# AbrahamSanders/realtime-codec-agent

Measured on AMD Instinct MI355X. Metric: batch-encode audio-hours/hour (+ xRT and p50 frame-step latency of 1 duplex stream in `duplex`), higher is better.
Workload: dtype f32; 1 GPU; batch MagiCodec-style encode, 16 kHz stereo, 0.1 s chunks / 2.0 s context, 256 windows per step (BASELINE configs[1]); codebook=131072x16

## Files before the change

### realtime_codec_agent_amd/csrc/rca_codec.hip

```cpp
#include <stdarg.h>

#include <algorithm>
#include <array>
#include <cmath>
#include <map>
#include <type_traits>

#include "rca_common.h"

namespace rca {
thread_local char g_err[512] = {0};
}
using namespace rca;

typedef float f32x16 __attribute__((ext_vector_type(16)));

#define RCA_LAT_MAX_FRAMES 64
#define RCA_LDS_BUDGET (152 * 1024)

typedef float f32x4 __attribute__((ext_vector_type(4)));

struct RowSrc {
    const float* base;
    int C;
// ... 1508 lines not shown
            cinit[4 * g + 0] = h4.x; cinit[4 * g + 1] = h4.y; cinit[4 * g + 2] = h4.z; cinit[4 * g + 3] = h4.w;
        }
#pragma unroll
        for (int ft = 0; ft < FN; ++ft) {
            f32x16 acc = cinit;
#pragma unroll
            for (int kp = 0; kp < 8; ++kp) acc = __builtin_amdgcn_mfma_f32_32x32x2f32(av[kp], zb[ft][kp], acc, 0, 0, 0);
#pragma unroll
            for (int r = 0; r < 16; ++r) {
                const unsigned c = (unsigned)(c0 + (r & 3) + 8 * (r >> 2) + 4 * half);
                if (acc[r] > best[ft]) { best[ft] = acc[r]; bidx[ft] = c; }
            }
        }
    }
    __shared__ unsigned long long red[FN][4][32];
#pragma unroll
    for (int ft = 0; ft < FN; ++ft) {
        unsigned long long key = bidx[ft] == 0xFFFFFFFFu ? 0ull : pack_key(best[ft], bidx[ft]);
        const unsigned long long other = __shfl_xor(key, 32);
        key = other > key ? other : key;
        if (lane < 32) red[ft][wave][lane] = key;
    }
    __syncthreads();
    for (int i = threadIdx.x; i < FN * 32; i += 256) {
        const int ft = i >> 5, l = i & 31;
        const long f = f0 + i;
        if (f < F) {
            unsigned long long key = red[ft][0][l];
            for (int w = 1; w < 4; ++w) key = red[ft][w][l] > key ? red[ft][w][l] : key;
            atomicMax(&keys[f], key);
        }
    }
}

struct RowDst {
    int64_t* base;
    int C;
    long chan_stride;
    long win_stride;
    int fc;
    const long* row_off = nullptr;
};
__global__ __launch_bounds__(256) void vq_finalize_kernel(unsigned long long* __restrict__ keys, RowDst dst, long rows) {
    const long i = (long)blockIdx.x * blockDim.x + threadIdx.x;
    if (i >= rows) return;
    const unsigned long long key = keys[i];
    keys[i] = 0ull;
    const long b = i / dst.fc;
    const int j = (int)(i - b * dst.fc);
    dst.base[(dst.row_off ? dst.row_off[b] : (b % dst.C) * dst.chan_stride + (b / dst.C) * dst.win_stride) + j] =
        key == 0ull ? (int64_t)0 : (int64_t)(0xFFFFFFFFu - (unsigned)(key & 0xFFFFFFFFull));
}

__global__ __launch_bounds__(256) void embed_codes_kernel(const int64_t* __restrict__ codes, long ldc, const float* __restrict__ cb,
                                                          float* __restrict__ zq, int B, int F, int J, int N,
                                                          int* __restrict__ err) {
    const long idx = (long)blockIdx.x * blockDim.x + threadIdx.x;
    if (idx >= (long)B * J * F) return;
    const int f = (int)(idx % F);
    const long r = idx / F;
    const int j = (int)(r % J);
    const int b = (int)(r / J);
    int64_t c = codes[(long)b * ldc + f];
    if (c < 0 || c >= N) { atomicExch(err, 1); c = 0; }
    zq[idx] = cb[c * J + j];
}

__global__ __launch_bounds__(256) void transpose_fj_kernel(const float* __restrict__ in, float* __restrict__ out, int B,
                                                           int F, int J) {
    const long idx = (long)blockIdx.x * blockDim.x + threadIdx.x;
    if (idx >= (long)B * J * F) return;
    const int f = (int)(idx % F);
    const long r = idx / F;
    const int j = (int)(r % J);
    const int b = (int)(r / J);
    out[idx] = in[((long)b * F + f) * J + j];
}
__global__ __launch_bounds__(256) void transpose_df_kernel(const float* __restrict__ in, float* __restrict__ out, int B,
                                                           int D, int F) {
    const long idx = (long)blockIdx.x * blockDim.x + threadIdx.x;
    if (idx >= (long)B * D * F) return;
    const int d = (int)(idx % D);
    const long r = idx / D;
    const int f = (int)(r % F);
    const int b = (int)(r / F);
    out[idx] = in[((long)b * D + d) * F + f];
}

struct ConvLayer {
    int cin, cout, k, s, pre, tr;
    float* w = nullptr;
    float* b = nullptr;
    float* bp = nullptr;
    float* wp = nullptr;
    int K = 0, Kpad = 0, cout_pad = 0, nchunks = 0;
    float* wp2 = nullptr;
    int nchunks2 = 0;
    float* wp_tr = nullptr;
    float* w_lat = nullptr;
    int nchunks_tr = 0;
};

#ifdef RCA_CONV_SMALLCHUNK
#define RCA_CIC_K8 2
#define RCA_CIC_K16 1
#else
// ... 297 lines not shown
    return;
#endif
#pragma unroll
    for (int wn = 0; wn < 4; ++wn)
#pragma unroll
    for (int wm = 0; wm < WMT; ++wm) {
        const int t = n0 + wn_w * 128 + wn * 32 + n;
        if (t >= Lout) continue;
        if (OUT == 1) {
            float* yr = y_f32 + ((long)b * Cout + co0 + wm * 32 + 4 * half) * Lout + t;
#pragma unroll
            for (int r = 0; r < 16; ++r) yr[(long)((r & 3) + 8 * (r >> 2)) * Lout] = acc[wm][wn][r];
        } else {
            const int Cbo = Cout / 16;
#pragma unroll
            for (int g = 0; g < 4; ++g) {
                float v[4];
#pragma unroll
                for (int j = 0; j < 4; ++j) {
                    const float a = acc[wm][wn][4 * g + j];
                    v[j] = act ? fmaxf(a, a * slope) : a;
                }
                const int ch = co0 + wm * 32 + 8 * g + 4 * half;
                const long o = (((long)b * Cbo + ch / 16) * Lout + t) * 16 + (ch & 15);
                const unsigned h0 = conv_pack_bf16x2(v[0], v[1]), h1 = conv_pack_bf16x2(v[2], v[3]);
                *reinterpret_cast<uint2*>(y_hi + o) = make_uint2(h0, h1);
                if (SPLIT) {
                    const unsigned l0 = conv_pack_bf16x2(v[0] - __uint_as_float(h0 << 16), v[1] - __uint_as_float(h0 & 0xffff0000u));
                    const unsigned l1 = conv_pack_bf16x2(v[2] - __uint_as_float(h1 << 16), v[3] - __uint_as_float(h1 & 0xffff0000u));
                    *reinterpret_cast<uint2*>(y_lo + o) = make_uint2(l0, l1);
                }
            }
        }
    }
}

struct Bf16Pack { conv_bf16raw* hi = nullptr; conv_bf16raw* lo = nullptr; float* w_in8 = nullptr; };

struct rca_codec {
    rca_codec_config_t cfg;
    int device = 0;
    hipStream_t stream = nullptr;
    int hop = 1;
    int variant = 1;
    int mfma_mode = 0;
    bool lat_mode = false;
    int enc_left_frames = 0, dec_left_frames = 0;
    bool window_trim = false;
    std::vector<ConvLayer> enc, dec;
    std::vector<Bf16Pack> bf16_packs;
    bool bf16_blk_split = true;
    float *q_in_w = nullptr, *q_in_b = nullptr;
    float *cb = nullptr, *hc = nullptr, *cbp = nullptr;
    DevBuf act[2], zbuf, keys, io_a, io_b, tail;
    void* pin = nullptr; size_t pin_cap = 0;
    struct StreamGraph { hipGraphExec_t exec = nullptr; int seen = 0; unsigned long long sig = 0; };
    std::map<std::array<int, 5>, StreamGraph> sgraphs;
    bool stream_graphs = true;
    int* err_flag = nullptr;
    hipStream_t last_stream = nullptr;
    bool last_stream_valid = false;
    hipEvent_t xev = nullptr;
    struct Prof { hipEvent_t a, b; int kclass; double flops, bytes; };
    bool profile = false;
    std::vector<Prof> prof;
    std::vector<Prof> prof_pool;
};

struct ProfScope {
    rca_codec* h; hipStream_t st; rca_codec::Prof p; bool on;
    ProfScope(rca_codec* h_, hipStream_t st_, int kclass, double flops, double bytes) : h(h_), st(st_), on(h_->profile) {
        if (!on) return;
        if (!h->prof_pool.empty()) { p = h->prof_pool.back(); h->prof_pool.pop_back(); }
        else { (void)hipEventCreate(&p.a); (void)hipEventCreate(&p.b); }
        p.kclass = kclass; p.flops = flops; p.bytes = bytes;
        (void)hipEventRecord(p.a, st);
    }
    ~ProfScope() {
        if (!on) return;
        (void)hipEventRecord(p.b, st);
        h->prof.push_back(p);
    }
};

static int upload(const rca_tensor_t* ts, int n, const std::string& name, long numel, float** out) {
    const rca_tensor_t* t = find_tensor(ts, n, name);
    if (!t) return fail(RCA_ERR_MISSING, "tensor '%s' missing", name.c_str());
    if (t->numel != numel) return fail(RCA_ERR_ARG, "tensor '%s': numel %ld, expected %ld", name.c_str(), (long)t->numel, numel);
    if (t->dtype != RCA_F32) return fail(RCA_ERR_ARG, "tensor '%s' must be f32", name.c_str());
    RCA_HIP(hipMalloc((void**)out, (size_t)numel * sizeof(float)));
    RCA_HIP(hipMemcpy(*out, t->data, (size_t)numel * sizeof(float), hipMemcpyHostToDevice));
    return RCA_OK;
}

static int pack_weights_cic(const float* w_host, const ConvLayer& L, int cic, float** out, int* nchunks_out) {
    const int K = L.cin * L.k;
    const int nchunks = (L.cin + cic - 1) / cic;
    const int Kpad = nchunks * cic * L.k;
    const int cout_pad = (L.cout + 127) / 128 * 128;
    const long n = (long)(cout_pad / 32) * (Kpad / 8) * 64 * 4;
    std::vector<float> p((size_t)n, 0.0f);
    for (int cot = 0; cot < cout_pad / 32; ++cot)
        for (int q = 0; q < Kpad / 8; ++q)
            for (int lane = 0; lane < 64; ++lane)
                for (int e = 0; e < 4; ++e) {
                    const int co = cot * 32 + (lane & 31);
                    const int k = 2 * (4 * q + e) + (lane >> 5);
// ... 56 lines not shown

extern "C" const char* rca_last_error(void) { return g_err; }
extern "C" const char* rca_version(void) { return "rca-hip 0.1 (gfx950)"; }
extern "C" int rca_device_sync(int32_t device) {
    RCA_HIP(hipSetDevice(device));
    RCA_HIP(hipDeviceSynchronize());
    return RCA_OK;
}

extern "C" int rca_device_count(int* n) {
    if (!n) return fail(RCA_ERR_ARG, "null");
    RCA_HIP(hipGetDeviceCount(n));
    return RCA_OK;
}

extern "C" int rca_codec_destroy(rca_codec_t* h) {
#ifdef RCA_CONV_TIMELINE
    if (h && getenv("RCA_CONV_TIMELINE_OUT")) {
        long* b = nullptr;
        unsigned n = 6 << 16;
        (void)hipDeviceSynchronize();
        (void)hipMemcpyFromSymbol(&b, HIP_SYMBOL(rca_prof_buf), 8);
        if (b) {
            std::vector<long> host((size_t)(6 << 16) * 8);
            (void)hipMemcpy(host.data(), b, host.size() * 8, hipMemcpyDeviceToHost);
            if (FILE* f = fopen(getenv("RCA_CONV_TIMELINE_OUT"), "wb")) { fwrite(&n, 4, 1, f); fwrite(host.data(), 8, host.size(), f); fclose(f); }
        }
    }
#endif

    if (!h) return RCA_OK;
    (void)hipSetDevice(h->device);
    for (auto& pk : h->bf16_packs) {
        if (pk.hi) (void)hipFree(pk.hi);
        if (pk.lo) (void)hipFree(pk.lo);
        if (pk.w_in8) (void)hipFree(pk.w_in8);
    }
    for (auto* v : {&h->enc, &h->dec})
        for (auto& L : *v) {
            if (L.w) (void)hipFree(L.w);
            if (L.b) (void)hipFree(L.b);
            if (L.bp) (void)hipFree(L.bp);
            if (L.wp) (void)hipFree(L.wp);
            if (L.wp2) (void)hipFree(L.wp2);
            if (L.wp_tr) (void)hipFree(L.wp_tr);
            if (L.w_lat) (void)hipFree(L.w_lat);
        }
    for (float* p : {h->q_in_w, h->q_in_b, h->cb, h->hc, h->cbp})
        if (p) (void)hipFree(p);
    if (h->err_flag) (void)hipFree(h->err_flag);
    for (auto& kv : h->sgraphs)
        if (kv.second.exec) (void)hipGraphExecDestroy(kv.second.exec);
    if (h->pin) (void)hipHostFree(h->pin);
    h->act[0].release(); h->act[1].release(); h->zbuf.release(); h->keys.release(); h->io_a.release(); h->io_b.release(); h->tail.release();
    for (auto* v : {&h->prof, &h->prof_pool})
        for (auto& p : *v) { (void)hipEventDestroy(p.a); (void)hipEventDestroy(p.b); }
    if (h->xev) (void)hipEventDestroy(h->xev);
    if (h->stream) (void)hipStreamDestroy(h->stream);
    delete h;
    return RCA_OK;
}

static void codec_receptive_field(const rca_codec_config_t& c, int hop, int* enc_left, int* dec_left) {
    const int n = c.n_stages;
    long lo = 0;
    lo = lo - (c.k_latent - 1 + 1) / 2;
    for (int i = n - 1; i >= 0; --i) { const int s = c.strides[i], k = 2 * s; lo = lo * s - (k - s + 1) / 2; }
    lo = lo - (c.k_in - 1 + 1) / 2;
    *enc_left = (int)((-lo + hop - 1) / hop);
    auto ceil_div = [](long a, long b) { return a >= 0 ? (a + b - 1) / b : -((-a) / b); };
    long u = 0;
    u = u - (c.k_in - 1 + 1) / 2;
    for (int i = 0; i < n; ++i) { const int s = c.strides[i], k = 2 * s; u = ceil_div(u + (k - s + 1) / 2 - (k - 1), s); }
    u = u - (c.k_latent - 1 + 1) / 2;
    *dec_left = (int)(-u);
}

extern "C" int rca_codec_create(const rca_codec_config_t* cfg, const rca_tensor_t* ts, int32_t nt, int32_t device,
                                rca_codec_t** out) {
    if (!cfg || !ts || !out) return fail(RCA_ERR_ARG, "null argument");
    if (cfg->n_stages < 1 || cfg->n_stages > RCA_MAX_STAGES) return fail(RCA_ERR_ARG, "n_stages out of range");
    if (cfg->codebook_dim != 16) return fail(RCA_ERR_ARG, "codebook_dim must be 16 (got %d)", cfg->codebook_dim);
    if (cfg->codebook_size % 128 != 0) return fail(RCA_ERR_ARG, "codebook_size must be a multiple of 128");
    if (cfg->k_in != 7 && cfg->k_in != 3 && cfg->k_in != 5) return fail(RCA_ERR_ARG, "k_in must be 3, 5 or 7");
    if (!(cfg->leaky_slope > 0.0f && cfg->leaky_slope < 1.0f)) return fail(RCA_ERR_ARG, "leaky_slope must be in (0, 1)");
    RCA_HIP(hipSetDevice(device));
    rca_codec* h = new rca_codec();
    h->cfg = *cfg;
    h->device = device;
    int rc = RCA_OK;
    auto bail = [&](int code) { rca_codec_destroy(h); return code; };
    if (hipStreamCreateWithFlags(&h->stream, hipStreamNonBlocking) != hipSuccess) return bail(fail(RCA_ERR_HIP, "stream create"));
    const int n = cfg->n_stages;
    h->hop = 1;
    for (int i = 0; i < n; ++i) h->hop *= cfg->strides[i];
    codec_receptive_field(*cfg, h->hop, &h->enc_left_frames, &h->dec_left_frames);

    auto add = [&](std::vector<ConvLayer>& v, const std::string& name, int cin, int cout, int k, int s, int pre, int tr,
                   bool pack) -> int {
        ConvLayer L;
        L.cin = cin; L.cout = cout; L.k = k; L.s = s; L.pre = pre; L.tr = tr;
        if ((rc = upload(ts, nt, name + ".weight", (long)cin * cout * k, &L.w)) != RCA_OK) return rc;
        if ((rc = upload(ts, nt, name + ".bias", cout, &L.b)) != RCA_OK) { v.push_back(L); return rc; }
        {
            const size_t nb = ((size_t)cout + 127) / 128 * 128 + 64;
            if (hipMalloc((void**)&L.bp, nb * 4) != hipSuccess || hipMemset(L.bp, 0, nb * 4) != hipSuccess ||
                hipMemcpy(L.bp, L.b, (size_t)cout * 4, hipMemcpyDeviceToDevice) != hipSuccess) {
// ... 507 lines not shown
        const int Lout = L / E1.s;
        {
            ProfScope ps(h, st, 0, 2.0 * E1.cin * E1.k * E1.cout * (double)B * Lout + 2.0 * E0.k * E0.cout * (double)B * L,
                         4.0 * ((double)B * src.T + (double)B * E1.cout * Lout + (double)E1.cin * E1.k * E1.cout));
            prev_post = handoff(2, Lout);
            const int act = (E1.pre ? 1 : 0) | (prev_post ? 2 : 0);
            if (h->variant == 2 && try_conv_ws(E1, nullptr, y, B, L, Lout, slope, st, &fin)) { rc = RCA_OK; RCA_LAUNCH_CHECK(); }
            else if (E1.k == 4) rc = launch_conv_mfma<4, 2, 4>(E1, nullptr, y, B, L, Lout, slope, st, &fin, act, h->mfma_mode);
            else if (E1.k == 8) rc = launch_conv_mfma<8, 4, RCA_CIC_K8>(E1, nullptr, y, B, L, Lout, slope, st, &fin, act, h->mfma_mode);
            else rc = launch_conv_mfma<16, 8, RCA_CIC_K16>(E1, nullptr, y, B, L, Lout, slope, st, &fin, act, h->mfma_mode);
        }
        if (rc != RCA_OK) return rc;
        L = Lout;
        first = 2;
        if (tap_layer == 1) RCA_HIP(hipMemcpyAsync(tap_dev, y, (size_t)B * E1.cout * L * 4, hipMemcpyDeviceToDevice, st));
    } else if (h->lat_mode && !src.row_off && src.win_stride == 0 && src.C == B &&
               try_conv_lds(h, h->enc[0], src.base, src.chan_stride, src.T, h->act[cur].as<float>(), B, L, 0, st)) {
        RCA_LAUNCH_CHECK();
    } else {
        const ConvLayer& L0 = h->enc[0];
        const long total = (long)B * L;
        float* y = h->act[cur].as<float>();
        ProfScope ps(h, st, 2, 2.0 * L0.k * L0.cout * (double)total, 4.0 * ((double)total + (double)total * L0.cout));
        if (L0.k == 7) conv_in_kernel<7><<<cdiv(total, 256), 256, 0, st>>>(src, L0.w, L0.b, y, B, L0.cout, L);
        else if (L0.k == 5) conv_in_kernel<5><<<cdiv(total, 256), 256, 0, st>>>(src, L0.w, L0.b, y, B, L0.cout, L);
        else conv_in_kernel<3><<<cdiv(total, 256), 256, 0, st>>>(src, L0.w, L0.b, y, B, L0.cout, L);
        RCA_LAUNCH_CHECK();
        if (tap_layer == 0) RCA_HIP(hipMemcpyAsync(tap_dev, y, (size_t)B * L0.cout * L * 4, hipMemcpyDeviceToDevice, st));
    }
    for (size_t li = first; li < h->enc.size(); ++li) {
        const ConvLayer& Ly = h->enc[li];
        float* x = h->act[cur].as<float>();
        float* y = h->act[cur ^ 1].as<float>();
        bool done = false;
        int view = 0;
        if (li + 1 == h->enc.size() && Fz_out && keep > 0 && tap_layer < 0 && !Ly.tr) {
            const char* hk = getenv("RCA_HEAD_KEEP");
            const int want = keep + conv_view_halo(Ly);
            if (!(hk && hk[0] == '0') && want < L / Ly.s && conv_view_ok(h, Ly, B, L, want)) view = want;
        }
        if ((rc = run_conv(h, Ly, x, y, B, L, 0, st, prev_post, handoff(li + 1, L / Ly.s), &done, view)) != RCA_OK) return rc;
        if (view) *Fz_out = view;
        prev_post = done;
        L /= Ly.s;
        cur ^= 1;
        if (tap_layer == (int)li) RCA_HIP(hipMemcpyAsync(tap_dev, y, (size_t)B * Ly.cout * L * 4, hipMemcpyDeviceToDevice, st));
    }
    *ze_out = h->act[cur].as<float>();
    *F_out = F;
    return RCA_OK;
}

static int run_quantize(rca_codec* h, const float* ze, int ze_is_rows, int B, int F, int f0, int fc, RowDst dst, hipStream_t st,
                        float* ztap_dev) {
    const rca_codec_config_t& c = h->cfg;
    const long rows = (long)B * fc;
    const int J = c.codebook_dim, N = c.codebook_size;
    int rc;
    if ((rc = h->zbuf.ensure((size_t)rows * J * 4)) != RCA_OK) return rc;
    const size_t need_keys = (size_t)rows;
    if (h->keys.cap < need_keys * 8) {
        if ((rc = h->keys.ensure(need_keys * 8)) != RCA_OK) return rc;
        RCA_HIP(hipMemsetAsync(h->keys.p, 0, h->keys.cap, st));
    }
    float* z = h->zbuf.as<float>();
    in_proj_kernel<<<cdiv(rows * J, 256), 256, 0, st>>>(ze, h->q_in_w, h->q_in_b, z, B, c.latent_dim, F, f0, fc, J, ze_is_rows);
    RCA_LAUNCH_CHECK();
    if (ztap_dev) RCA_HIP(hipMemcpyAsync(ztap_dev, z, (size_t)rows * J * 4, hipMemcpyDeviceToDevice, st));
    unsigned long long* keys = h->keys.as<unsigned long long>();
    ProfScope ps(h, st, 1, 2.0 * (double)rows * N * J, 4.0 * ((double)N * (J + 1) + (double)rows * J) + 8.0 * rows);
    if (h->variant >= 1) {
        constexpr int FN = 2;
        const int ftiles = (int)cdiv(rows, FN * 32);
        const int total_tiles = N / 32;
        int splits = (int)std::max(1L, std::min((long)total_tiles / 16, (1024 + ftiles - 1) / (long)ftiles));
        int tps = (total_tiles + splits - 1) / splits;
        tps = (tps + 3) / 4 * 4;
        splits = (total_tiles + tps - 1) / tps;
        dim3 grid(ftiles, splits);
        vq_mfma_kernel<FN><<<grid, 256, 0, st>>>(z, h->cbp, h->hc, keys, rows, N, tps);
    } else {
        constexpr int FB = 4;
        const int fblocks = (int)cdiv(rows, FB);
        int splits = (int)std::max(1L, std::min((long)N / 1024, (1024 + fblocks - 1) / (long)fblocks));
        int cps = (N + splits - 1) / splits;
        cps = (cps + 255) / 256 * 256;
        splits = (N + cps - 1) / cps;
        dim3 grid(fblocks, splits);
        vq_chain_kernel<FB><<<grid, 256, 0, st>>>(z, h->cb, h->hc, keys, rows, N, cps);
    }
    RCA_LAUNCH_CHECK();
    dst.fc = fc;
    vq_finalize_kernel<<<cdiv(rows, 256), 256, 0, st>>>(keys, dst, rows);
    RCA_LAUNCH_CHECK();
    return RCA_OK;
}

static hipStream_t pick_stream(rca_codec* h, void* stream) {
    hipStream_t st = (hipStream_t)stream;
    if (h->last_stream_valid && h->last_stream != st) {
        if (!h->xev) (void)hipEventCreateWithFlags(&h->xev, hipEventDisableTiming);
        (void)hipEventRecord(h->xev, h->last_stream);
        (void)hipStreamWaitEvent(st, h->xev, 0);
    }
    h->last_stream = st;
    h->last_stream_valid = true;
    return st;
}

extern "C" int rca_codec_encode_dev(rca_codec_t* h, const float* pcm, int32_t B, int32_t T, int64_t* codes, void* stream) {
    if (!h || !pcm || !codes || B < 1 || T < 1) return fail(RCA_ERR_ARG, "encode: bad argument (B=%d T=%d)", B, T);
    RCA_HIP(hipSetDevice(h->device));
    hipStream_t st = pick_stream(h, stream);
    RowSrc src{pcm, B, (long)T, 0, T};
    float* ze; int F, rc;
    if ((rc = run_encoder(h, src, B, st, &ze, &F, -1, nullptr)) != RCA_OK) return rc;
    RowDst dst{codes, B, (long)F, 0, F};
    return run_quantize(h, ze, 0, B, F, 0, F, dst, st, nullptr);
}

static int trimmable_frames(const rca_codec* h, int F, int keep) { return std::max(0, F - keep - h->enc_left_frames); }

extern "C" int rca_codec_encode_tail_dev(rca_codec_t* h, const float* pcm, int32_t B, int32_t T, int32_t n_keep, int64_t* codes,
                                         void* stream) {
    if (!h || !pcm || !codes || B < 1 || T < 1 || n_keep < 1) return fail(RCA_ERR_ARG, "encode_tail: bad argument (B=%d T=%d keep=%d)", B, T, n_keep);
    const int F = (T + h->hop - 1) / h->hop;
    if (n_keep > F) return fail(RCA_ERR_ARG, "encode_tail: %d frames wanted, the window holds %d", n_keep, F);
    RCA_HIP(hipSetDevice(h->device));
    hipStream_t st = pick_stream(h, stream);
    const int j = trimmable_frames(h, F, n_keep);
    RowSrc src{pcm + (long)j * h->hop, B, (long)T, 0, T - j * h->hop};
    float* ze; int Ft, rc;
    h->lat_mode = h->variant >= 1 && (long)B * (F - j) <= RCA_LAT_MAX_FRAMES;
    int Fz;
    rc = run_encoder(h, src, B, st, &ze, &Ft, -1, nullptr, -1, nullptr, n_keep, &Fz);
    h->lat_mode = false;
    if (rc != RCA_OK) return rc;
    RowDst dst{codes, B, (long)n_keep, 0, n_keep};
    return run_quantize(h, ze, 0, B, Fz, Fz - n_keep, n_keep, dst, st, nullptr);
}

extern "C" int rca_codec_receptive_field(const rca_codec_t* h, int32_t* enc_left_frames, int32_t* dec_left_frames) {
    if (!h || !enc_left_frames || !dec_left_frames) return fail(RCA_ERR_ARG, "null");
    *enc_left_frames = h->enc_left_frames;
    *dec_left_frames = h->dec_left_frames;
    return RCA_OK;
}

extern "C" int rca_codec_set_window_trim(rca_codec_t* h, int32_t enable) {
    if (!h) return fail(RCA_ERR_ARG, "null");
    h->window_trim = enable != 0;
    return RCA_OK;
}

extern "C" int rca_codec_encode(rca_codec_t* h, const float* pcm_host, int32_t B, int32_t T, int64_t* codes_host) {
    if (!h || !pcm_host || !codes_host || B < 1 || T < 1) return fail(RCA_ERR_ARG, "encode: bad argument (B=%d T=%d)", B, T);
    RCA_HIP(hipSetDevice(h->device));
    const int F = (T + h->hop - 1) / h->hop;
    int rc;
    if ((rc = h->io_a.ensure((size_t)B * T * 4)) != RCA_OK) return rc;
    if ((rc = h->io_b.ensure((size_t)B * F * 8)) != RCA_OK) return rc;
    RCA_HIP(hipMemcpyAsync(h->io_a.p, pcm_host, (size_t)B * T * 4, hipMemcpyHostToDevice, h->stream));
    if ((rc = rca_codec_encode_dev(h, h->io_a.as<float>(), B, T, h->io_b.as<int64_t>(), h->stream)) != RCA_OK) return rc;
    RCA_HIP(hipMemcpyAsync(codes_host, h->io_b.p, (size_t)B * F * 8, hipMemcpyDeviceToHost, h->stream));
    RCA_HIP(hipStreamSynchronize(h->stream));
    return RCA_OK;
}

extern "C" int rca_codec_encode_tap(rca_codec_t* h, const float* pcm_host, int32_t B, int32_t T, int32_t layer, float* out_host,
                                    int64_t out_numel) {
    if (!h || !pcm_host || !out_host || B < 1 || T < 1) return fail(RCA_ERR_ARG, "tap: bad argument");
    RCA_HIP(hipSetDevice(h->device));
    const int n = h->cfg.n_stages;
    if (layer < 0 || layer > n + 2) return fail(RCA_ERR_ARG, "tap layer out of range");
    int rc;
    if ((rc = h->io_a.ensure((size_t)B * T * 4)) != RCA_OK) return rc;
    if ((rc = h->io_b.ensure((size_t)out_numel * 4)) != RCA_OK) return rc;
    RCA_HIP(hipMemcpyAsync(h->io_a.p, pcm_host, (size_t)B * T * 4, hipMemcpyHostToDevice, h->stream));
    RowSrc src{h->io_a.as<float>(), B, (long)T, 0, T};
    float* ze; int F;
    (void)pick_stream(h, h->stream);
    {
        const int Fx = (T + h->hop - 1) / h->hop;
        long L = (long)Fx * h->hop, want;
        if (layer == 0) want = (long)B * h->cfg.channels[0] * L;
        else if (layer <= n) { for (int i = 0; i < layer; ++i) L /= h->cfg.strides[i]; want = (long)B * h->cfg.channels[layer] * L; }
        else if (layer == n + 1) want = (long)B * h->cfg.latent_dim * Fx;
        else want = (long)B * Fx * h->cfg.codebook_dim;
        if (want != out_numel) return fail(RCA_ERR_ARG, "tap: out_numel %ld, expected %ld", (long)out_numel, want);
    }
    if ((rc = run_encoder(h, src, B, h->stream, &ze, &F, layer <= n + 1 ? layer : -1, h->io_b.as<float>())) != RCA_OK) return rc;
    if (layer == n + 2) {
// ... 15 lines not shown
                                         uint16_t* lo_host, int64_t numel) {
    if (!h || !pcm_host || !hi_host || B < 1 || T < 1) return fail(RCA_ERR_ARG, "bf16 tap: bad argument");
    RCA_HIP(hipSetDevice(h->device));
    const int n = h->cfg.n_stages;
    if (layer < 0 || layer > n) return fail(RCA_ERR_ARG, "bf16 tap: layer %d out of range", layer);
    {
        long L = (long)((T + h->hop - 1) / h->hop) * h->hop;
        for (int i = 0; i < layer; ++i) L /= h->cfg.strides[i];
        const long want = (long)B * h->cfg.channels[layer] * L;
        if (want != numel) return fail(RCA_ERR_ARG, "bf16 tap: numel %ld, expected %ld", (long)numel, want);
    }
    int rc;
    if ((rc = h->io_a.ensure((size_t)B * T * 4)) != RCA_OK) return rc;
    RCA_HIP(hipMemcpyAsync(h->io_a.p, pcm_host, (size_t)B * T * 4, hipMemcpyHostToDevice, h->stream));
    RowSrc src{h->io_a.as<float>(), B, (long)T, 0, T};
    (void)pick_stream(h, h->stream);
    float* ze; int F;
    const conv_bf16raw* planes[2] = {nullptr, nullptr};
    if ((rc = run_encoder(h, src, B, h->stream, &ze, &F, -1, nullptr, layer, planes)) != RCA_OK) return rc;
    RCA_HIP(hipMemcpyAsync(hi_host, planes[0], (size_t)numel * 2, hipMemcpyDeviceToHost, h->stream));
    if (h->mfma_mode == 3 && lo_host) RCA_HIP(hipMemcpyAsync(lo_host, planes[1], (size_t)numel * 2, hipMemcpyDeviceToHost, h->stream));
    RCA_HIP(hipStreamSynchronize(h->stream));
    return RCA_OK;
}

extern "C" int rca_codec_encode_chunk_range_dev(rca_codec_t* h, const float* audio, int32_t C, int64_t N, int32_t chunk, int32_t ctx,
                                                int32_t batch_windows, int64_t chunk_begin, int64_t chunk_end, int64_t* codes,
                                                int64_t codes_per_channel, void* stream) {
    if (!h || !audio || !codes || C < 1 || N < 1 || chunk < 1 || ctx < 0 || batch_windows < 1)
        return fail(RCA_ERR_ARG, "encode_windows: bad argument");
    RCA_HIP(hipSetDevice(h->device));
    hipStream_t st = pick_stream(h, stream);
    const int sr = h->cfg.sample_rate;
    const double framerate = (double)sr / (double)h->hop;
    const int fpc = (int)(((double)chunk / (double)sr) * framerate);
    const long n_chunks = N / chunk;
    if (chunk_begin < 0 || chunk_end > n_chunks || chunk_begin > chunk_end)
        return fail(RCA_ERR_ARG, "chunk range [%ld,%ld) outside [0,%ld]", (long)chunk_begin, (long)chunk_end, n_chunks);
    if (fpc < 1) return fail(RCA_ERR_ARG, "chunk of %d samples holds no whole frame", chunk);
    if (codes_per_channel < (chunk_end - chunk_begin) * fpc)
        return fail(RCA_ERR_ARG, "codes buffer too small: %ld < %ld", (long)codes_per_channel, (long)(chunk_end - chunk_begin) * fpc);
    const int W = std::max(chunk, ctx);
    int rc;
    long i = chunk_begin;
    for (; i < chunk_end && (i + 1) * (long)chunk < W; ++i) {
        const int Tfull = (int)((i + 1) * chunk);
        const int jw = h->window_trim ? trimmable_frames(h, (Tfull + h->hop - 1) / h->hop, fpc) : 0;
        const int T = Tfull - jw * h->hop;
        RowSrc src{audio + (long)jw * h->hop, C, (long)N, 0, T};
        float* ze; int F, Fz;
        if ((rc = run_encoder(h, src, C, st, &ze, &F, -1, nullptr, -1, nullptr, fpc, &Fz)) != RCA_OK) return rc;
        if (F < fpc) return fail(RCA_ERR_STATE, "window of %d samples has %d frames < %d kept", T, F, fpc);
        RowDst dst{codes + (i - chunk_begin) * fpc, C, (long)codes_per_channel, 0, fpc};
        if ((rc = run_quantize(h, ze, 0, C, Fz, Fz - fpc, fpc, dst, st, nullptr)) != RCA_OK) return rc;
    }
    const int wins_per_pass = std::max(1, batch_windows / C);
    while (i < chunk_end) {
        const int nw = (int)std::min<long>(wins_per_pass, chunk_end - i);
        const int jw = h->window_trim ? trimmable_frames(h, (W + h->hop - 1) / h->hop, fpc) : 0;
        const long start0 = (i + 1) * (long)chunk - W + (long)jw * h->hop;
        RowSrc src{audio + start0, C, (long)N, (long)chunk, W - jw * h->hop};
        float* ze; int F, Fz;
        if ((rc = run_encoder(h, src, nw * C, st, &ze, &F, -1, nullptr, -1, nullptr, fpc, &Fz)) != RCA_OK) return rc;
        if (F < fpc) return fail(RCA_ERR_STATE, "window has %d frames < %d kept", F, fpc);
        RowDst dst{codes + (i - chunk_begin) * fpc, C, (long)codes_per_channel, (long)fpc, fpc};
        if ((rc = run_quantize(h, ze, 0, nw * C, Fz, Fz - fpc, fpc, dst, st, nullptr)) != RCA_OK) return rc;
        i += nw;
    }
    return RCA_OK;
}

extern "C" int rca_codec_encode_windows_dev(rca_codec_t* h, const float* audio, int32_t C, int64_t N, int32_t chunk, int32_t ctx,
                                            int32_t batch_windows, int64_t* codes, int64_t codes_per_channel, void* stream) {
    if (chunk < 1) return fail(RCA_ERR_ARG, "encode_windows: bad argument");
    return rca_codec_encode_chunk_range_dev(h, audio, C, N, chunk, ctx, batch_windows, 0, N / chunk, codes, codes_per_channel, stream);
}

extern "C" int rca_codec_encode_rows_dev(rca_codec_t* h, const float* audio, const int64_t* src_off, int32_t B, int32_t T, int32_t n_keep,
                                         int64_t* codes, const int64_t* dst_off, int64_t span, void* stream) {
    if (!h || !audio || !src_off || !codes || !dst_off || B < 1 || T < 1 || n_keep < 1 || span < T)
        return fail(RCA_ERR_ARG, "encode_rows: bad argument");
    RCA_HIP(hipSetDevice(h->device));
    hipStream_t st = pick_stream(h, stream);
    static_assert(sizeof(long) == sizeof(int64_t), "offset tables are 64-bit");
    const int Ffull = (T + h->hop - 1) / h->hop;
    if (Ffull < n_keep) return fail(RCA_ERR_ARG, "encode_rows: a window of %d samples has %d frames < %d kept", T, Ffull, n_keep);
    const int jw = h->window_trim ? trimmable_frames(h, Ffull, n_keep) : 0;
    RowSrc src{audio + (long)jw * h->hop, B, 0, 0, T - jw * h->hop, reinterpret_cast<const long*>(src_off), (long)span};
    float* ze; int F, Fz;
    int rc;
    if ((rc = run_encoder(h, src, B, st, &ze, &F, -1, nullptr, -1, nullptr, n_keep, &Fz)) != RCA_OK) return rc;
    RowDst dst{codes, B, 0, 0, n_keep, reinterpret_cast<const long*>(dst_off)};
    return run_quantize(h, ze, 0, B, Fz, Fz - n_keep, n_keep, dst, st, nullptr);
}

extern "C" int rca_codec_encoder_dev(rca_codec_t* h, const float* pcm, int32_t B, int32_t T, float* ze_out, void* stream) {
    if (!h || !pcm || !ze_out || B < 1 || T < 1) return fail(RCA_ERR_ARG, "encoder: bad argument");
    RCA_HIP(hipSetDevice(h->device));
    hipStream_t st = pick_stream(h, stream);
    RowSrc src{pcm, B, (long)T, 0, T};
    float* ze; int F, rc;
    if ((rc = run_encoder(h, src, B, st, &ze, &F, -1, nullptr)) != RCA_OK) return rc;
    const long total = (long)B * h->cfg.latent_dim * F;
    transpose_df_kernel<<<cdiv(total, 256), 256, 0, st>>>(ze, ze_out, B, h->cfg.latent_dim, F);
    RCA_LAUNCH_CHECK();
    return RCA_OK;
}

extern "C" int rca_codec_quantize_dev(rca_codec_t* h, const float* ze_rows, int64_t rows, int64_t* codes, void* stream) {
    if (!h || !ze_rows || !codes || rows < 1) return fail(RCA_ERR_ARG, "quantize: bad argument");
    RCA_HIP(hipSetDevice(h->device));
    hipStream_t st = pick_stream(h, stream);
    RowDst dst{codes, 1, 0, (long)rows, (int)rows};
    return run_quantize(h, ze_rows, 1, 1, (int)rows, 0, (int)rows, dst, st, nullptr);
}

static int run_decoder(rca_codec* h, float* zq , int B, int F, float* pcm_out, hipStream_t st) {
    const rca_codec_config_t& c = h->cfg;
    int rc;
    int cur = 0;
    int L = F;
    for (size_t li = 0; li < h->dec.size(); ++li) {
        const ConvLayer& Ly = h->dec[li];
        const bool last = li + 1 == h->dec.size();
        float* x = h->act[cur].as<float>();
        float* y = last ? pcm_out : h->act[cur ^ 1].as<float>();
        if ((rc = run_conv(h, Ly, x, y, B, L, last ? 1 : 0, st)) != RCA_OK) return rc;
        if (Ly.tr) L *= Ly.s;
        cur ^= 1;
    }
    (void)c; (void)zq;
    return RCA_OK;
}

static int decoder_workspace(rca_codec* h, int B, int F) {
    const rca_codec_config_t& c = h->cfg;
    const int n = c.n_stages;
    size_t max_elems = (size_t)B * c.codebook_dim * F;
    long L = F;
    max_elems = std::max(max_elems, (size_t)B * c.channels[n] * L);
    for (int i = 0; i < n; ++i) { L *= c.strides[n - 1 - i]; max_elems = std::max(max_elems, (size_t)B * c.channels[n - 1 - i] * L); }
    int rc;
    if ((rc = h->act[0].ensure(max_elems * 4)) != RCA_OK) return rc;
    return h->act[1].ensure(max_elems * 4);
}

extern "C" int rca_codec_decode_dev(rca_codec_t* h, const int64_t* codes, int32_t B, int32_t F, float* pcm, void* stream) {
    if (!h || !codes || !pcm || B < 1 || F < 1) return fail(RCA_ERR_ARG, "decode: bad argument (B=%d F=%d)", B, F);
    RCA_HIP(hipSetDevice(h->device));
    hipStream_t st = pick_stream(h, stream);
    int rc;
    if ((rc = decoder_workspace(h, B, F)) != RCA_OK) return rc;
    const int J = h->cfg.codebook_dim;
    float* zq = h->act[0].as<float>();
    embed_codes_kernel<<<cdiv((long)B * J * F, 256), 256, 0, st>>>(codes, (long)F, h->cb, zq, B, F, J, h->cfg.codebook_size, h->err_flag);
    RCA_LAUNCH_CHECK();
    return run_decoder(h, zq, B, F, pcm, st);
}

extern "C" int rca_codec_decode_tail_dev(rca_codec_t* h, const int64_t* codes, int32_t B, int32_t F, int32_t n_samples, float* pcm,
                                         void* stream) {
    if (!h || !codes || !pcm || B < 1 || F < 1 || n_samples < 1) return fail(RCA_ERR_ARG, "decode_tail: bad argument (B=%d F=%d n=%d)", B, F, n_samples);
    if ((long)n_samples > (long)F * h->hop) return fail(RCA_ERR_ARG, "decode_tail: %d samples wanted, %d codes give %ld", n_samples, F, (long)F * h->hop);
    RCA_HIP(hipSetDevice(h->device));
    hipStream_t st = pick_stream(h, stream);
    const int f0 = (int)(((long)F * h->hop - n_samples) / h->hop);
    const int j = std::max(0, f0 - h->dec_left_frames);
    const int Ft = F - j;
    int rc;
    if ((rc = decoder_workspace(h, B, Ft)) != RCA_OK) return rc;
    const long Tt = (long)Ft * h->hop;
    if ((rc = h->tail.ensure((size_t)B * Tt * 4)) != RCA_OK) return rc;
    const int J = h->cfg.codebook_dim;
    float* zq = h->act[0].as<float>();
    embed_codes_kernel<<<cdiv((long)B * J * Ft, 256), 256, 0, st>>>(codes + j, (long)F, h->cb, zq, B, Ft, J, h->cfg.codebook_size, h->err_flag);
    RCA_LAUNCH_CHECK();
    h->lat_mode = h->variant >= 1 && (long)B * Ft <= RCA_LAT_MAX_FRAMES;
    rc = run_decoder(h, zq, B, Ft, h->tail.as<float>(), st);
    h->lat_mode = false;
    if (rc != RCA_OK) return rc;
    RCA_HIP(hipMemcpy2DAsync(pcm, (size_t)n_samples * 4, h->tail.as<float>() + (Tt - n_samples), (size_t)Tt * 4, (size_t)n_samples * 4, B,
                             hipMemcpyDeviceToDevice, st));
    return RCA_OK;
}

static unsigned long long workspace_signature(const rca_codec* h) {
    unsigned long long sig = 1469598103934665603ull;
    for (const void* p : {h->act[0].p, h->act[1].p, h->zbuf.p, h->keys.p, h->io_a.p, h->io_b.p, h->tail.p, (void*)h->pin}) {
        sig ^= (unsigned long long)(uintptr_t)p;
        sig *= 1099511628211ull;
    }
    return sig;
}
static int ensure_pinned(rca_codec* h, size_t bytes) {
    if (bytes <= h->pin_cap) return RCA_OK;
    if (h->pin) (void)hipHostFree(h->pin);
    h->pin = nullptr; h->pin_cap = 0;
    RCA_HIP(hipHostMalloc(&h->pin, bytes + (bytes >> 2), hipHostMallocDefault));
    h->pin_cap = bytes + (bytes >> 2);
    return RCA_OK;
}
static int stream_call(rca_codec* h, int kind, int B, int a, int b, const void* in_host, size_t in_bytes, void* out_host, size_t out_bytes) {
    RCA_HIP(hipSetDevice(h->device));
    hipStream_t st = h->stream;
    int rc;
    const size_t in_pad = (in_bytes + 255) & ~(size_t)255, out_pad = (out_bytes + 255) & ~(size_t)255;
    if ((rc = ensure_pinned(h, in_pad + out_pad + 256)) != RCA_OK) return rc;
    if ((rc = h->io_a.ensure(in_pad)) != RCA_OK) return rc;
    if ((rc = h->io_b.ensure(out_pad)) != RCA_OK) return rc;
    char* pin = (char*)h->pin;
    int* perr = (int*)(pin + in_pad + out_pad);
    memcpy(pin, in_host, in_bytes);
    auto enqueue = [&]() -> int {
        hipError_t e = hipMemcpyAsync(h->io_a.p, pin, in_bytes, hipMemcpyHostToDevice, st);
        if (e != hipSuccess) return fail(RCA_ERR_HIP, "stream h2d: %s", hipGetErrorString(e));
        int r = kind == 0 ? rca_codec_encode_tail_dev(h, h->io_a.as<float>(), B, a, b, h->io_b.as<int64_t>(), st)
                          : rca_codec_decode_tail_dev(h, h->io_a.as<int64_t>(), B, a, b, h->io_b.as<float>(), st);
        if (r != RCA_OK) return r;
        e = hipMemcpyAsync(pin + in_pad, h->io_b.p, out_bytes, hipMemcpyDeviceToHost, st);
        if (e == hipSuccess) e = hipMemcpyAsync(perr, h->err_flag, 4, hipMemcpyDeviceToHost, st);
        if (e != hipSuccess) return fail(RCA_ERR_HIP, "stream d2h: %s", hipGetErrorString(e));
        return RCA_OK;
    };
    (void)pick_stream(h, st);
    rca_codec::StreamGraph& g = h->sgraphs[{kind, B, a, b, h->variant}];
    const bool want_graph = h->stream_graphs && !h->profile && g.seen >= 1;
    if (want_graph && g.exec && g.sig != workspace_signature(h)) { (void)hipGraphExecDestroy(g.exec); g.exec = nullptr; }
    if (want_graph && !g.exec) {
        hipGraph_t graph = nullptr;
        RCA_HIP(hipStreamSynchronize(st));
        RCA_HIP(hipStreamBeginCapture(st, hipStreamCaptureModeThreadLocal));
        rc = enqueue();
        hipError_t e = hipStreamEndCapture(st, &graph);
        if (rc != RCA_OK) { if (graph) (void)hipGraphDestroy(graph); return rc; }
        if (e != hipSuccess) return fail(RCA_ERR_HIP, "stream capture: %s", hipGetErrorString(e));
        e = hipGraphInstantiate(&g.exec, graph, nullptr, nullptr, 0);
        (void)hipGraphDestroy(graph);
        if (e != hipSuccess) { g.exec = nullptr; return fail(RCA_ERR_HIP, "stream graph instantiate: %s", hipGetErrorString(e)); }
        g.sig = workspace_signature(h);
    }
    if (want_graph) {
// ... 135 lines not shown
```

Measured before the change: 3449 audio-hours/hour.

## Fuse VQ argmax finalize and rescoring into head kernel, add slab in-proj

Replaces the MFMA VQ search plus separate finalize with a kernel that tracks only the best 32-code tile per frame. The last split block, chosen by a per-row-tile atomic ticket, then rescores that tile's 32 codes in exact fp32 and writes the int64 codes directly. A second kernel loads the encoder output view and the transposed projection weights into LDS so each batch row's in-projection runs in one block. Both are meant to cut kernel launches and global traffic, at the cost of extra atomics and fences, a ticket buffer, and a rescoring tail that runs only in the last block.

```diff
diff --git a/realtime_codec_agent_amd/csrc/rca_codec.hip b/realtime_codec_agent_amd/csrc/rca_codec.hip
--- a/realtime_codec_agent_amd/csrc/rca_codec.hip
+++ b/realtime_codec_agent_amd/csrc/rca_codec.hip
@@ -1584,6 +1584,160 @@
         key == 0ull ? (int64_t)0 : (int64_t)(0xFFFFFFFFu - (unsigned)(key & 0xFFFFFFFFull));
 }
 
+template <int FN>
+__global__ __launch_bounds__(256, 2) void vq_head_kernel(const float* __restrict__ z, const float* __restrict__ cbp,
+                                                      const float* __restrict__ hc, const float* __restrict__ cb,
+                                                      unsigned long long* __restrict__ keys, unsigned* __restrict__ tickets,
+                                                      RowDst dst, long F, int N, int tiles_per_split) {
+    const int lane = threadIdx.x & 63;
+    const int wave = __builtin_amdgcn_readfirstlane(threadIdx.x >> 6);
+    const long f0 = (long)blockIdx.x * (FN * 32);
+    const int tile_beg = blockIdx.y * tiles_per_split;
+    const int tile_end = min(N / 32, tile_beg + tiles_per_split);
+    const int half = lane >> 5;
+
+    float zb[FN][8];
+#pragma unroll
+    for (int ft = 0; ft < FN; ++ft) {
+        const long f = f0 + ft * 32 + (lane & 31);
+#pragma unroll
+        for (int kp = 0; kp < 8; ++kp) zb[ft][kp] = f < F ? z[f * 16 + 2 * kp + half] : 0.0f;
+    }
+    float best[FN];
+    unsigned btile[FN];
+#pragma unroll
+    for (int ft = 0; ft < FN; ++ft) { best[ft] = -INFINITY; btile[ft] = 0xFFFFFFFFu; }
+
+    for (int tile = tile_beg + wave; tile < tile_end; tile += 4) {
+        const float4* ap = reinterpret_cast<const float4*>(cbp) + ((long)tile * 2) * 64 + lane;
+        const float4 a0 = ap[0], a1 = ap[64];
+        const float av[8] = {a0.x, a0.y, a0.z, a0.w, a1.x, a1.y, a1.z, a1.w};
+        const int c0 = tile * 32;
+        f32x16 cinit;
+#pragma unroll
+        for (int g = 0; g < 4; ++g) {
+            const float4 h4 = *reinterpret_cast<const float4*>(hc + c0 + 8 * g + 4 * half);
+            cinit[4 * g + 0] = h4.x; cinit[4 * g + 1] = h4.y; cinit[4 * g + 2] = h4.z; cinit[4 * g + 3] = h4.w;
+        }
+#pragma unroll
+        for (int ft = 0; ft < FN; ++ft) {
+            f32x16 acc = cinit;
+#pragma unroll
+            for (int kp = 0; kp < 8; ++kp) acc = __builtin_amdgcn_mfma_f32_32x32x2f32(av[kp], zb[ft][kp], acc, 0, 0, 0);
+            float t[5];
+#pragma unroll
+            for (int g = 0; g < 5; ++g) t[g] = __builtin_fmaxf(__builtin_fmaxf(acc[3 * g], acc[3 * g + 1]), acc[3 * g + 2]);
+            float m = __builtin_fmaxf(__builtin_fmaxf(t[0], t[1]), t[2]);
+            m = __builtin_fmaxf(__builtin_fmaxf(m, t[3]), t[4]);
+            m = __builtin_fmaxf(m, acc[15]);
+            const bool up = m > best[ft];
+            best[ft] = up ? m : best[ft];
+            btile[ft] = up ? (unsigned)tile : btile[ft];
+        }
+    }
+    __shared__ unsigned long long red[FN][4][32];
+    __shared__ unsigned last_ticket;
+#pragma unroll
+    for (int ft = 0; ft < FN; ++ft) {
+        unsigned long long key = btile[ft] == 0xFFFFFFFFu ? 0ull : pack_key(best[ft], btile[ft]);
+        const unsigned long long other = __shfl_xor(key, 32);
+        key = other > key ? other : key;
+        if (lane < 32) red[ft][wave][lane] = key;
+    }
+    __syncthreads();
+    for (int i = threadIdx.x; i < FN * 32; i += 256) {
+        const int ft = i >> 5, l = i & 31;
+        const long f = f0 + i;
+        if (f < F) {
+            unsigned long long key = red[ft][0][l];
+            for (int w = 1; w < 4; ++w) key = red[ft][w][l] > key ? red[ft][w][l] : key;
+            atomicMax(&keys[f], key);
+        }
+    }
+    __threadfence();
+    __syncthreads();
+    if (threadIdx.x == 0) last_ticket = atomicAdd(&tickets[blockIdx.x], 1u) == gridDim.y - 1 ? 1u : 0u;
+    __syncthreads();
+    if (!last_ticket) return;
+    __threadfence();
+    if (threadIdx.x == 0) atomicExch(&tickets[blockIdx.x], 0u);
+    for (int i0 = 0; i0 < FN * 32 * 4; i0 += 256) {
+        const int i = i0 + threadIdx.x;
+        const long f = f0 + (i >> 2);
+        const int q = i & 3;
+        unsigned long long key = 0ull;
+        if (q == 0 && f < F) key = atomicExch(&keys[f], 0ull);
+        key = __shfl(key, lane & ~3);
+        float sbest = -INFINITY;
+        unsigned sidx = 0xFFFFFFFFu;
+        if (key != 0ull) {
+            const unsigned cq = (0xFFFFFFFFu - (unsigned)(key & 0xFFFFFFFFull)) * 32u + 8u * q;
+            const float4* zp = reinterpret_cast<const float4*>(z + f * 16);
+            const float4 z0 = zp[0], z1 = zp[1], z2 = zp[2], z3 = zp[3];
+            const float zr[16] = {z0.x, z0.y, z0.z, z0.w, z1.x, z1.y, z1.z, z1.w, z2.x, z2.y, z2.z, z2.w, z3.x, z3.y, z3.z, z3.w};
+#pragma unroll
+            for (int e = 0; e < 8; ++e) {
+                const unsigned c = cq + e;
+                const float4* cr = reinterpret_cast<const float4*>(cb + (long)c * 16);
+                const float4 c0 = cr[0], c1 = cr[1], c2 = cr[2], c3 = cr[3];
+                const float cv[16] = {c0.x, c0.y, c0.z, c0.w, c1.x, c1.y, c1.z, c1.w, c2.x, c2.y, c2.z, c2.w, c3.x, c3.y, c3.z, c3.w};
+                float a = hc[c];
+#pragma unroll
+                for (int j = 0; j < 16; ++j) a = __builtin_fmaf(zr[j], cv[j], a);
+                if (a > sbest) { sbest = a; sidx = c; }
+            }
+        }
+        unsigned long long k2 = sidx == 0xFFFFFFFFu ? 0ull : pack_key(sbest, sidx);
+        unsigned long long o2 = __shfl_xor(k2, 1);
+        k2 = o2 > k2 ? o2 : k2;
+        o2 = __shfl_xor(k2, 2);
+        k2 = o2 > k2 ? o2 : k2;
+        if (q == 0 && f < F) {
+            const long b = f / dst.fc;
+            const int j = (int)(f - b * dst.fc);
+            dst.base[(dst.row_off ? dst.row_off[b] : (b % dst.C) * dst.chan_stride + (b / dst.C) * dst.win_stride) + j] =
+                k2 == 0ull ? (int64_t)0 : (int64_t)(0xFFFFFFFFu - (unsigned)(k2 & 0xFFFFFFFFull));
+        }
+    }
+}
+
+__global__ __launch_bounds__(256) void in_proj_slab_kernel(const float* __restrict__ ze, const float* __restrict__ w,
+                                                           const float* __restrict__ bias, float* __restrict__ z, int D,
+                                                           int F, int f0, int fc, int J) {
+    extern __shared__ float slab[];
+    float* zs = slab;
+    float* ws = slab + D * F;
+    const int b = blockIdx.x;
+    const float* zr = ze + (long)b * D * F;
+    const int nz = D * F, nw = J * D, JP = J + 1;
+    for (int i0 = 0; i0 < nz; i0 += 8 * 256) {
+        float v[8];
+#pragma unroll
+        for (int u = 0; u < 8; ++u) { const int i = i0 + u * 256 + (int)threadIdx.x; v[u] = zr[min(i, nz - 1)]; }
+#pragma unroll
+        for (int u = 0; u < 8; ++u) { const int i = i0 + u * 256 + (int)threadIdx.x; if (i < nz) zs[i] = v[u]; }
+    }
+    for (int i0 = 0; i0 < nw; i0 += 8 * 256) {
+        float v[8];
+#pragma unroll
+        for (int u = 0; u < 8; ++u) { const int i = i0 + u * 256 + (int)threadIdx.x; v[u] = w[min(i, nw - 1)]; }
+#pragma unroll
+        for (int u = 0; u < 8; ++u) {
+            const int i = i0 + u * 256 + (int)threadIdx.x;
+            if (i < nw) { const int j = i / D; ws[(i - j * D) * JP + j] = v[u]; }
+        }
+    }
+    __syncthreads();
+    for (int o = threadIdx.x; o < fc * J; o += 256) {
+        const int j = o % J;
+        const float* zc = zs + f0 + o / J;
+        const float* wc = ws + j;
+        float acc = bias[j];
+        for (int d = 0; d < D; ++d) acc = __builtin_fmaf(wc[d * JP], zc[d * F], acc);
+        z[(long)b * fc * J + o] = acc;
+    }
+}
+
 __global__ __launch_bounds__(256) void embed_codes_kernel(const int64_t* __restrict__ codes, long ldc, const float* __restrict__ cb,
                                                           float* __restrict__ zq, int B, int F, int J, int N,
                                                           int* __restrict__ err) {
@@ -1987,7 +2141,7 @@
     bool bf16_blk_split = true;
     float *q_in_w = nullptr, *q_in_b = nullptr;
     float *cb = nullptr, *hc = nullptr, *cbp = nullptr;
-    DevBuf act[2], zbuf, keys, io_a, io_b, tail;
+    DevBuf act[2], zbuf, keys, tickets, io_a, io_b, tail;
     void* pin = nullptr; size_t pin_cap = 0;
     struct StreamGraph { hipGraphExec_t exec = nullptr; int seen = 0; unsigned long long sig = 0; };
     std::map<std::array<int, 5>, StreamGraph> sgraphs;
@@ -2150,7 +2304,7 @@
     for (auto& kv : h->sgraphs)
         if (kv.second.exec) (void)hipGraphExecDestroy(kv.second.exec);
     if (h->pin) (void)hipHostFree(h->pin);
-    h->act[0].release(); h->act[1].release(); h->zbuf.release(); h->keys.release(); h->io_a.release(); h->io_b.release(); h->tail.release();
+    h->act[0].release(); h->act[1].release(); h->zbuf.release(); h->keys.release(); h->tickets.release(); h->io_a.release(); h->io_b.release(); h->tail.release();
     for (auto* v : {&h->prof, &h->prof_pool})
         for (auto& p : *v) { (void)hipEventDestroy(p.a); (void)hipEventDestroy(p.b); }
     if (h->xev) (void)hipEventDestroy(h->xev);
@@ -2764,7 +2918,7 @@
 }
 
 static int run_quantize(rca_codec* h, const float* ze, int ze_is_rows, int B, int F, int f0, int fc, RowDst dst, hipStream_t st,
-                        float* ztap_dev) {
+                        float* ztap_dev, bool ze_view = false) {
     const rca_codec_config_t& c = h->cfg;
     const long rows = (long)B * fc;
     const int J = c.codebook_dim, N = c.codebook_size;
@@ -2776,7 +2930,13 @@
         RCA_HIP(hipMemsetAsync(h->keys.p, 0, h->keys.cap, st));
     }
     float* z = h->zbuf.as<float>();
-    in_proj_kernel<<<cdiv(rows * J, 256), 256, 0, st>>>(ze, h->q_in_w, h->q_in_b, z, B, c.latent_dim, F, f0, fc, J, ze_is_rows);
+    const char* hf = getenv("RCA_HEAD_FUSED");
+    const bool fused = !(hf && hf[0] == '0');
+    const size_t slab_bytes = ((size_t)c.latent_dim * F + (size_t)c.latent_dim * (J + 1)) * 4;
+    if (fused && ze_view && !ze_is_rows && slab_bytes <= 48 * 1024 && (long)fc * J <= 4096)
+        in_proj_slab_kernel<<<B, 256, slab_bytes, st>>>(ze, h->q_in_w, h->q_in_b, z, c.latent_dim, F, f0, fc, J);
+    else
+        in_proj_kernel<<<cdiv(rows * J, 256), 256, 0, st>>>(ze, h->q_in_w, h->q_in_b, z, B, c.latent_dim, F, f0, fc, J, ze_is_rows);
     RCA_LAUNCH_CHECK();
     if (ztap_dev) RCA_HIP(hipMemcpyAsync(ztap_dev, z, (size_t)rows * J * 4, hipMemcpyDeviceToDevice, st));
     unsigned long long* keys = h->keys.as<unsigned long long>();
@@ -2790,6 +2950,16 @@
         tps = (tps + 3) / 4 * 4;
         splits = (total_tiles + tps - 1) / tps;
         dim3 grid(ftiles, splits);
+        if (fused && h->variant == 1 && J == 16 && N % 32 == 0) {
+            if (h->tickets.cap < (size_t)ftiles * 4) {
+                if ((rc = h->tickets.ensure((size_t)ftiles * 4)) != RCA_OK) return rc;
+                RCA_HIP(hipMemsetAsync(h->tickets.p, 0, h->tickets.cap, st));
+            }
+            dst.fc = fc;
+            vq_head_kernel<FN><<<grid, 256, 0, st>>>(z, h->cbp, h->hc, h->cb, keys, h->tickets.as<unsigned>(), dst, rows, N, tps);
+            RCA_LAUNCH_CHECK();
+            return RCA_OK;
+        }
         vq_mfma_kernel<FN><<<grid, 256, 0, st>>>(z, h->cbp, h->hc, keys, rows, N, tps);
     } else {
         constexpr int FB = 4;
@@ -2849,7 +3019,7 @@
     h->lat_mode = false;
     if (rc != RCA_OK) return rc;
     RowDst dst{codes, B, (long)n_keep, 0, n_keep};
-    return run_quantize(h, ze, 0, B, Fz, Fz - n_keep, n_keep, dst, st, nullptr);
+    return run_quantize(h, ze, 0, B, Fz, Fz - n_keep, n_keep, dst, st, nullptr, Fz < Ft);
 }
 
 extern "C" int rca_codec_receptive_field(const rca_codec_t* h, int32_t* enc_left_frames, int32_t* dec_left_frames) {
@@ -2971,7 +3141,7 @@
         if ((rc = run_encoder(h, src, C, st, &ze, &F, -1, nullptr, -1, nullptr, fpc, &Fz)) != RCA_OK) return rc;
         if (F < fpc) return fail(RCA_ERR_STATE, "window of %d samples has %d frames < %d kept", T, F, fpc);
         RowDst dst{codes + (i - chunk_begin) * fpc, C, (long)codes_per_channel, 0, fpc};
-        if ((rc = run_quantize(h, ze, 0, C, Fz, Fz - fpc, fpc, dst, st, nullptr)) != RCA_OK) return rc;
+        if ((rc = run_quantize(h, ze, 0, C, Fz, Fz - fpc, fpc, dst, st, nullptr, Fz < F)) != RCA_OK) return rc;
     }
     const int wins_per_pass = std::max(1, batch_windows / C);
     while (i < chunk_end) {
@@ -2983,7 +3153,7 @@
         if ((rc = run_encoder(h, src, nw * C, st, &ze, &F, -1, nullptr, -1, nullptr, fpc, &Fz)) != RCA_OK) return rc;
         if (F < fpc) return fail(RCA_ERR_STATE, "window has %d frames < %d kept", F, fpc);
         RowDst dst{codes + (i - chunk_begin) * fpc, C, (long)codes_per_channel, (long)fpc, fpc};
-        if ((rc = run_quantize(h, ze, 0, nw * C, Fz, Fz - fpc, fpc, dst, st, nullptr)) != RCA_OK) return rc;
+        if ((rc = run_quantize(h, ze, 0, nw * C, Fz, Fz - fpc, fpc, dst, st, nullptr, Fz < F)) != RCA_OK) return rc;
         i += nw;
     }
     return RCA_OK;
@@ -3010,7 +3180,7 @@
     int rc;
     if ((rc = run_encoder(h, src, B, st, &ze, &F, -1, nullptr, -1, nullptr, n_keep, &Fz)) != RCA_OK) return rc;
     RowDst dst{codes, B, 0, 0, n_keep, reinterpret_cast<const long*>(dst_off)};
-    return run_quantize(h, ze, 0, B, Fz, Fz - n_keep, n_keep, dst, st, nullptr);
+    return run_quantize(h, ze, 0, B, Fz, Fz - n_keep, n_keep, dst, st, nullptr, Fz < F);
 }
 
 extern "C" int rca_codec_encoder_dev(rca_codec_t* h, const float* pcm, int32_t B, int32_t T, float* ze_out, void* stream) {
@@ -3105,7 +3275,7 @@
 
 static unsigned long long workspace_signature(const rca_codec* h) {
     unsigned long long sig = 1469598103934665603ull;
-    for (const void* p : {h->act[0].p, h->act[1].p, h->zbuf.p, h->keys.p, h->io_a.p, h->io_b.p, h->tail.p, (void*)h->pin}) {
+    for (const void* p : {h->act[0].p, h->act[1].p, h->zbuf.p, h->keys.p, h->tickets.p, h->io_a.p, h->io_b.p, h->tail.p, (void*)h->pin}) {
         sig ^= (unsigned long long)(uintptr_t)p;
         sig *= 1099511628211ull;
     }
```

Result: slower. 3366 audio-hours/hour (-2.4%).
